# COMP6248-Reproducability-Challenge/selfsupervised-denoising

Hardware: AMD Instinct MI355X
Metric: training patches/sec (64x64 gauss25 SSDN) (higher is better)
Workload: dtype f16

## Files before the change

### selfsupervised-denoising_amd/csrc/conv_dma.hip

```cpp
#include "common.h"
#include <cstdlib>
#include <type_traits>
#include <utility>

#if defined(SSDN_CDMA_TUNING) || defined(SSDN_TUNING)
#define CD_ABL(xx, bit) (((xx).ablate & (bit)) != 0)
#define CD_TUNING 1
#else
#define CD_ABL(xx, bit) false
#define CD_TUNING 0
#endif

#ifndef CD_DEPHASE
#define CD_DEPHASE 0
#endif
#ifndef CD_MOVE_BARRIER
#define CD_MOVE_BARRIER 1
#endif
#ifndef CD_WARMUP
#define CD_WARMUP 1
#endif

namespace {

constexpr int CD_TBYTES = 31744;

struct CdAux {
    int m_base, m_cnt;
    int padT, padL, rev;
    int tiles_x, tiles_y;
    int segs, tps;
    int segs_sh;
    unsigned tx_magic;
    int nitems, xcd_map;
    int nfull, tail16;
    int ablate;
    int wrep;
    int dephase;
    unsigned long long* trace;
};

typedef __attribute__((address_space(3))) void* cd_lds_ptr;
__device__ __forceinline__ void dma16(unsigned lds_addr, int voff, __amdgpu_buffer_rsrc_t rs, int soff) {
    __builtin_amdgcn_raw_ptr_buffer_load_lds(rs, (cd_lds_ptr)(size_t)__builtin_amdgcn_readfirstlane(lds_addr), 16, voff, __builtin_amdgcn_readfirstlane(soff), 0, 0);
}

template <bool BF>
__device__ __forceinline__ void cd_mma(f32x16& c, half8 av, half8 bv) {
    if constexpr (BF) c = __builtin_amdgcn_mfma_f32_32x32x16_bf16(__builtin_bit_cast(bf16x8, av), __builtin_bit_cast(bf16x8, bv), c, 0, 0, 0);
    else c = __builtin_amdgcn_mfma_f32_32x32x16_f16(av, bv, c, 0, 0, 0);
}

template <int OFF>
__device__ __forceinline__ void lds_rd128(half8& dst, unsigned addr) {
    asm volatile("ds_read_b128 %0, %1 offset:%2" : "=v"(dst) : "v"(addr), "i"(OFF));
}
template <int MT>
__device__ __forceinline__ void lds_wait0(half8 (&aq)[MT], half8 (&bq)[2]) {
    if constexpr (MT == 3)
        asm volatile("s_waitcnt lgkmcnt(0)" : "+v"(aq[0]), "+v"(aq[1]), "+v"(aq[2]), "+v"(bq[0]), "+v"(bq[1]));
    else if constexpr (MT == 2)
        asm volatile("s_waitcnt lgkmcnt(0)" : "+v"(aq[0]), "+v"(aq[1]), "+v"(bq[0]), "+v"(bq[1]));
    else
        asm volatile("s_waitcnt lgkmcnt(0)" : "+v"(aq[0]), "+v"(bq[0]), "+v"(bq[1]));
}
template <int MT, int KS, int I, int J, int KS_>
__device__ __forceinline__ void cd_reads(half8 (&aq)[MT], half8 (&bq)[2], unsigned ap, unsigned bp) {
    constexpr int PSTR = KS * 32, PITCH = 18 * PSTR, BOFF = I * PITCH + J * PSTR;
    lds_rd128<BOFF + KS_ * 32>(bq[0], bp);
    lds_rd128<0 * 32 * PSTR + KS_ * 32>(aq[0], ap);
    lds_rd128<BOFF + 2 * PITCH + KS_ * 32>(bq[1], bp);
    if constexpr (MT > 1) lds_rd128<1 * 32 * PSTR + KS_ * 32>(aq[1], ap);
    if constexpr (MT > 2) lds_rd128<2 * 32 * PSTR + KS_ * 32>(aq[2], ap);
}
template <int MT, bool BF>
__device__ __forceinline__ void cd_mmas(f32x16 (&acc)[MT][2], const half8 (&aq)[MT], const half8 (&bq)[2]) {
#pragma unroll
    for (int mt = 0; mt < MT; ++mt) {
        cd_mma<BF>(acc[mt][0], aq[mt], bq[0]);
        cd_mma<BF>(acc[mt][1], aq[mt], bq[1]);
    }
}

struct CdTile { int n, y0, x0; };

template <int MT, bool FULL>
struct CdWSplit {
    static constexpr int nq = FULL ? MT * 3 : MT;
    static constexpr int NB = (nq + 1) / 2 > 4 ? 4 : (nq + 1) / 2;
    static constexpr bool extra = nq > 2 * NB;
    static constexpr int b1 = extra ? NB : nq - NB;
};
template <int N> using cd_ic = std::integral_constant<int, N>;
template <class F, int... Is>
__device__ __forceinline__ void cd_static_for_impl(F& f, std::integer_sequence<int, Is...>) { (f(cd_ic<Is>{}), ...); }
template <int N, class F>
__device__ __forceinline__ void cd_static_for(F&& f) { cd_static_for_impl(f, std::make_integer_sequence<int, N>{}); }
template <int IMM, int AUX = 0>
__device__ __forceinline__ void dma16i(unsigned lds_addr, int voff, __amdgpu_buffer_rsrc_t rs, int soff) {
    __builtin_amdgcn_raw_ptr_buffer_load_lds(rs, (cd_lds_ptr)(size_t)lds_addr, 16, voff, soff, IMM, AUX);
}

}

template <int MT, bool BF, int EPI, int KIND>
__global__ __launch_bounds__(256, 2) void k_cdma(ssdn_conv_args a, CdAux x) {
    constexpr bool AF = KIND == 1;
    extern __shared__ __attribute__((aligned(16))) char smem[];
    constexpr int WROWS = MT * 32;
    constexpr int WBYTES = WROWS * 96;
    constexpr int OSTR = MT * 64 + 16;
    constexpr int NEK = MT * 2;
    constexpr bool HAS_MASK = (EPI & 1) != 0, HAS_ADD = (EPI & 2) != 0, HAS_UPS = (EPI & 4) != 0, UROT = (EPI & 8) != 0;
    constexpr bool SOUT = (EPI & 16) != 0, SMASK = (EPI & 32) != 0;
    constexpr int NUK = (8 * MT * 4 + 63) / 64;
    constexpr int G = 2 * MT;
    constexpr bool MOVE = CD_MOVE_BARRIER != 0;
    const int tid = threadIdx.x, lane = tid & 63, l31 = lane & 31, kh = lane >> 5;
    const int w = __builtin_amdgcn_readfirstlane(tid >> 6);
    const bool wload = w < 2;
    const int lw = w & 1;
    const unsigned lds0 = (unsigned)(size_t)smem;
    char* const tbuf0 = smem;
    const unsigned tlds0 = lds0, wlds0 = lds0 + 2 * CD_TBYTES;

    const int G_ = gridDim.x;
    int it_first, it_stride, it_end;
    if (x.xcd_map) {
        const int i8 = x.nitems >> 3, xcd = blockIdx.x & 7;
        it_first = xcd * i8 + (blockIdx.x >> 3); it_stride = G_ >> 3; it_end = (xcd + 1) * i8;
    } else {
        it_first = blockIdx.x; it_stride = G_; it_end = x.nitems;
    }
    if (it_first >= it_end) return;
#if CD_WARMUP
    const int pf_line = (blockIdx.x >> 3) * 256 + tid;
    const unsigned pf = __builtin_amdgcn_raw_buffer_load_b32(
        __builtin_amdgcn_make_buffer_rsrc(const_cast<void*>(a.wc), 0, 9 * a.Mpad * a.Ktot * 2, SSDN_BUFFER_RSRC_FLAGS), pf_line << 7, 0, 0);
#endif

    const int bE48 = (4 * w + (l31 >> 4)) * 1728 + (l31 & 15) * 96 + ((kh ^ ((l31 >> 4) & 1)) << 4);
    const int aB48 = l31 * 96 + ((kh ^ ((l31 >> 3) & 1)) << 4);
    const int cpp = x.m_cnt >> 3;

    const __amdgpu_buffer_rsrc_t rs_wc = __builtin_amdgcn_make_buffer_rsrc(const_cast<void*>(a.wc), 0, (int)0x80000000, SSDN_BUFFER_RSRC_FLAGS);
    const int H0 = a.up0 ? (a.H >> 1) : a.H, W0 = a.up0 ? (a.W >> 1) : a.W;
    const int nch = x.nfull + x.tail16;

    int tr_i = 0;
    auto stamp = [&]() __attribute__((always_inline)) {
        if (CD_TUNING && x.trace && tid == 0 && tr_i < 32) x.trace[(size_t)blockIdx.x * 32 + tr_i++] = __builtin_amdgcn_s_memtime();
    };

    const int wtap = a.Mpad * a.Ktot * 2;
    const int wt0 = x.rev ? 8 * wtap : 0, wts = x.rev ? -wtap : wtap;
    const int wvoff = lane * 16;
    const bool lw0 = __builtin_amdgcn_readfirstlane(tid >> 6) == 0;
    auto wchunk = [&](int c) __attribute__((always_inline)) {
        return __builtin_amdgcn_readfirstlane((c * 48 * a.Mpad + x.m_base * ((AF || c < x.nfull) ? 48 : 16)) * 2 + wt0);
    };
    auto wpiece = [&](auto FULLc, auto Jc, unsigned d, int so) __attribute__((always_inline)) {
        using S = CdWSplit<MT, decltype(FULLc)::value != 0>;
        constexpr int j = decltype(Jc)::value;
        if (CD_ABL(x, 2)) return;
        if constexpr (j < S::NB) dma16i<j * 1024>(d, wvoff, rs_wc, so);
        else if constexpr (S::extra) { if (lw0) dma16i<0>(d + 2 * S::NB * 1024, wvoff, rs_wc, so + 2 * S::NB * 1024); }
    };
    auto wbase = [&](bool full) __attribute__((always_inline)) {
        return lw ? (full ? CdWSplit<MT, true>::b1 : CdWSplit<MT, false>::b1) * 1024 : 0;
    };
    auto wslice = [&](bool full, unsigned dbuf, int sl) __attribute__((always_inline)) {
        const int wb = wbase(full);
        if (AF || full) cd_static_for<CdWSplit<MT, true>::NB + 1>([&](auto jc) { wpiece(cd_ic<1>{}, jc, dbuf + wb, sl + wb); });
        else cd_static_for<CdWSplit<MT, false>::NB + 1>([&](auto jc) { wpiece(cd_ic<0>{}, jc, dbuf + wb, sl + wb); });
    };

    __amdgpu_buffer_rsrc_t rs_t = rs_wc;
    int t_so = 0, t_incA = 0, t_incB = 0, t_ybs = 0, rlE = 0, rlO = 0;
    unsigned t_tb = 0;
    auto tile_setup = [&](int tn, int ty0, int tx0, int c, int tbi, bool live) __attribute__((always_inline)) {
        const int k0 = c * 48;
        const bool from0 = k0 < a.c0;
        const bool up = from0 && a.up0;
        const int cs = from0 ? a.src0.cs : a.src1.cs;
        const int cbase = from0 ? a.src0.co + k0 : a.src1.co + k0 - a.c0;
        const int Hs = up ? H0 : a.H, Ws = up ? W0 : a.W;
        const bool full = AF || c < x.nfull;
        const int rstride = __builtin_amdgcn_readfirstlane(Ws * cs * 2);
        const int rbase = __builtin_amdgcn_readfirstlane(((CD_ABL(x, 128) ? 0 : tn) * Hs * Ws * cs + cbase) * 2);
        t_ybs = __builtin_amdgcn_readfirstlane(ty0 - x.padT);
        const int y_first = t_ybs + (full ? 0 : lw);
        t_so = rbase + (up ? y_first >> 1 : y_first) * rstride;
        t_incA = up ? ((y_first & 1) ? rstride : 0) : rstride;
        t_incB = up ? ((y_first & 1) ? 0 : rstride) : rstride;
        if (!full) { t_incA = up ? rstride : 2 * rstride; t_incB = t_incA; }
        t_tb = __builtin_amdgcn_readfirstlane(tlds0 + tbi * CD_TBYTES + (full ? lw * (44 * 16) : lw * 576));
        rs_t = __builtin_amdgcn_make_buffer_rsrc(from0 ? a.src0.p : (a.src1.p ? a.src1.p : a.src0.p), 0, live ? (int)0x80000000 : 0, SSDN_BUFFER_RSRC_FLAGS);
        const int rp = full ? lane + 44 * lw : lane;
        const int hp = rp / 6;
        const int hx = full ? hp : rp >> 1;
        const int cc = full ? rp - hp * 6 : rp & 1;
        const int xx = tx0 - x.padL + hx;
        const bool ok = (unsigned)xx < (unsigned)a.W;
        const int xs = up ? xx >> 1 : xx;
        rlE = ok ? (xs * cs + cc * 8) * 2 : (int)0x80000000;
        rlO = ok ? (xs * cs + (cc ^ 1) * 8) * 2 : (int)0x80000000;
    };
    auto trow = [&](auto FULLc, auto HYc) __attribute__((always_inline)) {
        constexpr bool full = decltype(FULLc)::value != 0;
        constexpr int hy = decltype(HYc)::value;
        if (CD_ABL(x, 4)) return;
        const int so = t_so;
        t_so += (hy & 1) ? t_incB : t_incA;
        if constexpr (full) {
            int voff = (hy & 1) ? rlO : rlE;
            if constexpr (hy < 2 || hy >= 16) voff = (unsigned)(t_ybs + hy) < (unsigned)a.H ? voff : (int)0x80000000;
            if (CD_ABL(x, 512)) dma16i<0, 2>(t_tb + hy * 1728, voff, rs_t, so);
            else dma16i<0>(t_tb + hy * 1728, voff, rs_t, so);
        } else {
            int voff = lw ? rlO : rlE;
            voff = (unsigned)(t_ybs + lw + 2 * hy) < (unsigned)a.H ? voff : (int)0x80000000;
            if (lane < 36) dma16i<0>(t_tb + hy * 1152, voff, rs_t, so);
        }
    };

    auto tile_of = [&](int item, int k) {
        const int strip = item >> x.segs_sh, seg = item & (x.segs - 1);
        CdTile t;
        t.n = x.tiles_x == 1 ? strip : (int)__umulhi((unsigned)strip, x.tx_magic);
        t.x0 = (strip - t.n * x.tiles_x) * 16;
        t.y0 = (seg * x.tps + k) * 16;
        return t;
    };
    int item = it_first, kt = 0;
    CdTile cur = tile_of(item, 0);
    int tpar = 0, wpar = 0;
    float* const bl = reinterpret_cast<float*>(smem + 18 * 18 * 96);
    if (tid < WROWS) bl[tid] = (a.bias && tid < x.m_cnt) ? a.bias[x.m_base + tid] : 0.f;
    constexpr int CD_LUT = 18 * 18 * 96 + 384;
    static_assert(CD_LUT + 256 <= CD_TBYTES && WROWS * 4 <= 384, "pad behind tile buffer 0");
    if constexpr (SMASK && HAS_MASK) {
        if (tid < 64) reinterpret_cast<float*>(smem + CD_LUT)[tid] = ((tid >> 2) >> (tid & 3)) & 1 ? 1.f : LRELU_SLOPE;
    }

    const __amdgpu_buffer_rsrc_t rs_dst = __builtin_amdgcn_make_buffer_rsrc(UROT ? a.urot.p : a.dst.p, 0, CD_ABL(x, 64) ? 0 : (int)0x80000000, SSDN_BUFFER_RSRC_FLAGS);
    const __amdgpu_buffer_rsrc_t rs_sgn = __builtin_amdgcn_make_buffer_rsrc(SOUT ? a.sign_out : a.urot_smask, 0, (!CD_ABL(x, 64) && (SOUT || (UROT && a.urot_smask))) ? (int)0x80000000 : 0, SSDN_BUFFER_RSRC_FLAGS);
    const __amdgpu_buffer_rsrc_t rs_ms = __builtin_amdgcn_make_buffer_rsrc(const_cast<void*>(HAS_UPS ? a.upsum_mask_sign : a.mask_sign), 0, SMASK ? (int)0x80000000 : 0, SSDN_BUFFER_RSRC_FLAGS);
    const float slope = a.act ? LRELU_SLOPE : 1.f;
    const __amdgpu_buffer_rsrc_t rs_mask = __builtin_amdgcn_make_buffer_rsrc(a.mask.p, 0, HAS_MASK ? (int)0x80000000 : 0, SSDN_BUFFER_RSRC_FLAGS);
    const __amdgpu_buffer_rsrc_t rs_add = __builtin_amdgcn_make_buffer_rsrc(a.add.p, 0, HAS_ADD ? (int)0x80000000 : 0, SSDN_BUFFER_RSRC_FLAGS);
    const __amdgpu_buffer_rsrc_t rs_up = __builtin_amdgcn_make_buffer_rsrc(a.upsum.p, 0, HAS_UPS ? (int)0x80000000 : 0, SSDN_BUFFER_RSRC_FLAGS);
    const __amdgpu_buffer_rsrc_t rs_um = __builtin_amdgcn_make_buffer_rsrc(a.upsum_mask.p, 0, HAS_UPS ? (int)0x80000000 : 0, SSDN_BUFFER_RSRC_FLAGS);
    int u_pc[NUK];
#pragma unroll
    for (int k = 0; k < NUK; ++k) {
        const int p = k * 64 + lane;
        const int j = p / cpp, c = p - j * cpp;
        u_pc[k] = p < 8 * cpp ? (j | (c << 8)) : -1;
    }

    auto run = [&](auto WLc) __attribute__((always_inline)) {
    constexpr bool WL = decltype(WLc)::value != 0;
    if constexpr (WL) {
        wslice(KIND != 0 || 0 < x.nfull, wlds0, wchunk(0));
        wslice(KIND != 0 || 0 < x.nfull, wlds0 + WBYTES, wchunk(0) + wts);
    } else {
        tile_setup(cur.n, cur.y0, cur.x0, 0, 0, true);
        if (KIND != 0 || 0 < x.nfull) cd_static_for<18>([&](auto hc) { trow(cd_ic<1>{}, hc); });
        else cd_static_for<9>([&](auto hc) { trow(cd_ic<0>{}, hc); });
    }
    asm volatile("s_waitcnt vmcnt(0)" ::: "memory");
    __builtin_amdgcn_s_barrier();
    if (CD_TUNING && x.trace && tid == 0) x.trace[(size_t)blockIdx.x * 32 + 31] = 0x100000000ull | (unsigned)__builtin_amdgcn_s_getreg((31 << 11) | 4);
    if (x.dephase > 0 && ((__builtin_amdgcn_s_getreg((31 << 11) | 4) >> 16) & 1))
        for (int d = 0; d < x.dephase; ++d) __builtin_amdgcn_s_sleep(16);
    stamp();
    for (;;) {
        int nitem = item, nkt = kt + 1;
        if (nkt >= x.tps) { nkt = 0; nitem = item + it_stride; }
        const bool has_next = nitem < it_end;
        const CdTile nxt = tile_of(has_next ? nitem : item, nkt);

        f32x16 acc[MT][2];
        int bo = kh * 16;
        asm volatile("" : "+v"(bo));
#pragma unroll
        for (int mt = 0; mt < MT; ++mt)
#pragma unroll
            for (int g = 0; g < 4; ++g) {
                const f32x4 bb = *reinterpret_cast<const f32x4*>(smem + 18 * 18 * 96 + (mt * 32 + g * 8) * 4 + bo);
#pragma unroll
                for (int j = 0; j < 4; ++j) { acc[mt][0][g * 4 + j] = bb[j]; acc[mt][1][g * 4 + j] = bb[j]; }
            }

        auto chunk = [&](int c, auto CFc, auto PFc) __attribute__((always_inline)) {
            constexpr int CF = decltype(CFc)::value, PFK = decltype(PFc)::value;
            const bool last_chunk = c + 1 == nch;
            const bool pf = !last_chunk || has_next;
            const int pc = last_chunk ? 0 : c + 1;
            const bool cfull = CF == 2 ? c < x.nfull : CF == 1, pf_full = PFK == 2 ? pc < x.nfull : PFK == 1;
            const unsigned tb = tlds0 + tpar * CD_TBYTES;
            int bE_ = bE48, aB_ = aB48;
            if (!cfull) {
                int lo = lane;
                asm volatile("" : "+v"(lo));
                const int l31o = lo & 31, kho = lo >> 5;
                bE_ = (4 * w + (l31o >> 4)) * 576 + (l31o & 15) * 32 + ((kho ^ ((l31o >> 4) & 1)) << 4);
                aB_ = l31o * 32 + ((kho ^ ((l31o >> 3) & 1)) << 4);
            }
            const unsigned bE = tb + bE_, bO = tb + (bE_ ^ 16);
            const unsigned apE = wlds0 + wpar * WBYTES + aB_, apO = wlds0 + (wpar ^ 1) * WBYTES + aB_;
            const bool wfirst = c == 0;
            int wso = 0;
            unsigned wdA = 0, wdB = 0;
            if constexpr (WL) {
                const int wb = wbase(cfull);
                wso = wchunk(c) + wb;
                wdA = __builtin_amdgcn_readfirstlane(wlds0 + wpar * WBYTES + wb);
                wdB = __builtin_amdgcn_readfirstlane(wlds0 + (wpar ^ 1) * WBYTES + wb);
            } else {
                tile_setup(last_chunk ? nxt.n : cur.n, last_chunk ? nxt.y0 : cur.y0, last_chunk ? nxt.x0 : cur.x0, pc, tpar ^ 1, pf);
            }
            auto body = [&](auto FULLc, auto PFULLc) __attribute__((always_inline)) {
                constexpr bool FULL = decltype(FULLc)::value != 0, PFULL = decltype(PFULLc)::value != 0;
                constexpr int KS = FULL ? 3 : 1;
                constexpr bool MV = MOVE && FULL && KIND != 0;
                half8 fa[2][MT], fb[2][2];
                auto gap = [&](auto Tc, auto Ic) __attribute__((always_inline)) {
                    constexpr int T = decltype(Tc)::value, i = decltype(Ic)::value;
                    if constexpr (WL) {
                        using S = CdWSplit<MT, FULL>;
                        constexpr int NP = S::NB + (S::extra ? 1 : 0);
                        if constexpr (T < 8) {
                            if constexpr (i == 0) wso += wts;
                            cd_static_for<NP>([&](auto jc) {
                                constexpr int j = decltype(jc)::value;
                                if constexpr ((j < G - 1 ? j : G - 1) == i) {
                                    if constexpr (T == 0) { if (!wfirst) wpiece(FULLc, jc, wdB, wso); }
                                    else wpiece(FULLc, jc, (T & 1) ? wdA : wdB, wso);
                                }
                            });
                        } else if constexpr (i == 0) {
                            if (pf) wslice(pf_full, wlds0 + (wpar ^ 1) * WBYTES, wchunk(pc));
                        }
                    } else {
                        constexpr int N = PFULL ? 18 : 9, NS = G >= 3 ? G : 3;
                        constexpr int k0 = T * NS, n = k0 >= N ? 0 : (N - k0 < NS ? N - k0 : NS);
                        cd_static_for<n>([&](auto kc) {
                            constexpr int k = decltype(kc)::value;
                            if constexpr ((k < G - 1 ? k : G - 1) == i) trow(PFULLc, cd_ic<k0 + k>{});
                        });
                    }
                };
// ... 4 lines not shown
                        if (wfirst && NEPI > 0 && cpp == 4 * MT && !CD_ABL(x, 8 | 1024)) asm volatile("s_waitcnt vmcnt(%0)" ::"n"(NEPI) : "memory");
                        else asm volatile("s_waitcnt vmcnt(0)" ::: "memory");
                    } else if (WL || T == 8) asm volatile("s_waitcnt vmcnt(0)" ::: "memory");
                    __builtin_amdgcn_s_barrier();
                };
                auto step = [&](auto Tc) __attribute__((always_inline)) {
                    constexpr int T = decltype(Tc)::value, I = T / 3, J = T % 3;
                    constexpr int P = MV ? (T & 1) : 0;
                    const unsigned ap = (T & 1) ? apO : apE, bp = (I & 1) ? bO : bE;
                    if constexpr (!MV || T == 0) cd_reads<MT, KS, I, J, 0>(fa[P], fb[P], ap, bp);
                    lds_wait0<MT>(fa[P], fb[P]);
                    if constexpr (KS > 1) cd_reads<MT, KS, I, J, 1>(fa[P ^ 1], fb[P ^ 1], ap, bp);
                    __builtin_amdgcn_sched_barrier(0);
                    cd_static_for<G>([&](auto ic) {
                        constexpr int i = decltype(ic)::value;
                        if (!CD_ABL(x, 1)) cd_mma<BF>(acc[i >> 1][i & 1], fa[P][i >> 1], fb[P][i & 1]);
                        __builtin_amdgcn_sched_barrier(0);
                        gap(Tc, ic);
                        __builtin_amdgcn_sched_barrier(0);
                    });
                    if constexpr (KS > 1) {
                        lds_wait0<MT>(fa[P ^ 1], fb[P ^ 1]);
                        cd_reads<MT, KS, I, J, 2>(fa[P], fb[P], ap, bp);
                        __builtin_amdgcn_sched_barrier(0);
                        if (!CD_ABL(x, 1)) cd_mmas<MT, BF>(acc, fa[P ^ 1], fb[P ^ 1]);
                        __builtin_amdgcn_sched_barrier(0);
                        lds_wait0<MT>(fa[P], fb[P]);
                        if constexpr (MV && T < 8) {
                            sync(Tc);
                            constexpr int T1 = T + 1, I1 = T1 / 3, J1 = T1 % 3;
                            cd_reads<MT, KS, I1, J1, 0>(fa[P ^ 1], fb[P ^ 1], (T1 & 1) ? apO : apE, (I1 & 1) ? bO : bE);
                            __builtin_amdgcn_sched_barrier(0);
                            if (!CD_ABL(x, 1)) cd_mmas<MT, BF>(acc, fa[P], fb[P]);
                            __builtin_amdgcn_sched_barrier(0);
                        } else {
                            if (!CD_ABL(x, 1)) cd_mmas<MT, BF>(acc, fa[P], fb[P]);
                            __builtin_amdgcn_sched_barrier(0);
                            sync(Tc);
                        }
                    } else sync(Tc);
                };
                step(cd_ic<0>{});
                stamp();
                cd_static_for<8>([&](auto tc) { step(cd_ic<decltype(tc)::value + 1>{}); });
            };
            if constexpr (CF != 2 && PFK != 2) body(cd_ic<CF>{}, cd_ic<PFK>{});
            else if constexpr (WL) {
                if (cfull) body(cd_ic<1>{}, cd_ic<1>{}); else body(cd_ic<0>{}, cd_ic<1>{});
            } else if (cfull) {
                if (pf_full) body(cd_ic<1>{}, cd_ic<1>{}); else body(cd_ic<1>{}, cd_ic<0>{});
            } else {
                if (pf_full) body(cd_ic<0>{}, cd_ic<1>{}); else body(cd_ic<0>{}, cd_ic<0>{});
            }
            tpar ^= 1; wpar ^= 1;
            stamp();
        };
        if constexpr (KIND == 1) {
            for (int c = 0; c < nch; ++c) chunk(c, cd_ic<1>{}, cd_ic<1>{});
        } else if constexpr (KIND == 2) {
            for (int c = 0; c + 1 < x.nfull; ++c) chunk(c, cd_ic<1>{}, cd_ic<1>{});
            chunk(x.nfull - 1, cd_ic<1>{}, cd_ic<0>{});
            chunk(x.nfull, cd_ic<0>{}, cd_ic<1>{});
        } else {
            for (int c = 0; c < nch; ++c) chunk(c, cd_ic<2>{}, cd_ic<2>{});
        }
        if constexpr (WL) {
            if (has_next) wslice(KIND != 0 || 0 < x.nfull, wlds0 + (wpar ^ 1) * WBYTES, wchunk(0) + wts);
        }
        if (!CD_ABL(x, 8) && !HAS_UPS && (cpp & 1) == 0 && !CD_ABL(x, 1024)) {
            const int pix_t = (cur.n * a.H + cur.y0 + 4 * w) * a.W + cur.x0;
            const int npair = __builtin_amdgcn_readfirstlane(cpp >> 1);
            int lane_o = lane;
            asm volatile("" : "+v"(lane_o));
            const int l31 = lane_o & 31, kh = lane_o >> 5;
            const int lrow = l31 >> 4, lcol = l31 & 15;
            const int lpix = lrow * a.W + lcol;
            int ur_base = 0, ur_iu = 0, ur_iv = 0, ur_ju = 0, ur_jv = 0;
            if constexpr (UROT) {
                const int Bq = a.N >> 2, P1 = a.H - 1;
                const int r = (cur.n >= Bq ? 1 : 0) + (cur.n >= 2 * Bq ? 1 : 0) + (cur.n >= 3 * Bq ? 1 : 0);
                ur_iu = r == 0 ? 1 : (r == 2 ? -1 : 0); ur_iv = r == 1 ? 1 : (r == 3 ? -1 : 0);
                ur_ju = r == 3 ? 1 : (r == 1 ? -1 : 0); ur_jv = r == 0 ? 1 : (r == 2 ? -1 : 0);
                const int i0 = r >= 2 ? P1 : 0, j0 = (r == 1 || r == 2) ? P1 : 0;
                ur_base = (((cur.n - r * Bq) * a.H + i0) * a.W + j0) * a.urot.cs + a.urot.co + r * a.M;
            }
            constexpr bool HOIST = HAS_MASK && SMASK && !HAS_ADD && !UROT;
            unsigned mbh[2][MT * 2];
            if constexpr (HOIST) {
#pragma unroll
                for (int nt = 0; nt < 2; ++nt) {
                    const int pix_p = pix_t + 2 * nt * a.W;
                    const int s_so = __builtin_amdgcn_readfirstlane(pix_p * (a.M >> 3) + (x.m_base >> 3));
#pragma unroll
                    for (int i = 0; i < MT * 2; ++i) {
                        if (i >= npair) break;
                        mbh[nt][i] = __builtin_amdgcn_raw_buffer_load_b8(rs_ms, lpix * (a.M >> 3) + kh + i * 2, s_so, 0);
                    }
                }
            }
            auto pass = [&](auto NtC, auto ActC) __attribute__((always_inline)) {
                constexpr int nt = decltype(NtC)::value;
                constexpr bool ACTC = decltype(ActC)::value != 0;
                const int pix_p = pix_t + 2 * nt * a.W;
                int d_lane, d_so = 0;
                bool live = true;
                if constexpr (UROT) {
                    const int u = cur.y0 + 4 * w + 2 * nt + lrow + 1, v = cur.x0 + lcol;
                    live = u < a.H;
                    const int dpx = (ur_iu * u + ur_iv * v) * a.W + ur_ju * u + ur_jv * v;
                    d_lane = live ? (ur_base + dpx * a.urot.cs + x.m_base) * 2 + kh * 16 : (int)0x80000000;
                } else {
                    d_lane = lpix * a.dst.cs * 2 + kh * 16;
                    d_so = __builtin_amdgcn_readfirstlane((pix_p * a.dst.cs + a.dst.co + x.m_base) * 2);
                }
                const int s_lane = live ? lpix * (a.M >> 3) + kh : (int)0x80000000;
                const int s_so = __builtin_amdgcn_readfirstlane(pix_p * (a.M >> 3) + (x.m_base >> 3));
                u32x4_t ab[MT * 2], mb[MT * 2];
#pragma unroll
                for (int i = 0; i < MT * 2; ++i) {
                    if (i >= npair) break;
                    if constexpr (HAS_ADD)
                        ab[i] = __builtin_amdgcn_raw_buffer_load_b128(rs_add, lpix * a.add.cs * 2 + kh * 16 + i * 32,
                                                                      __builtin_amdgcn_readfirstlane((pix_p * a.add.cs + a.add.co + x.m_base) * 2), 0);
                    if constexpr (HOIST)
                        mb[i][0] = mbh[nt][i];
                    else if constexpr (HAS_MASK && SMASK)
                        mb[i][0] = __builtin_amdgcn_raw_buffer_load_b8(rs_ms, s_lane + i * 2, s_so, 0);
                    else if constexpr (HAS_MASK)
                        mb[i] = __builtin_amdgcn_raw_buffer_load_b128(rs_mask, lpix * a.mask.cs * 2 + kh * 16 + i * 32,
                                                                      __builtin_amdgcn_readfirstlane((pix_p * a.mask.cs + a.mask.co + x.m_base) * 2), 0);
                }
#pragma unroll
                for (int mt = 0; mt < MT; ++mt)
#pragma unroll
                    for (int gp = 0; gp < 2; ++gp) {
                        constexpr int DUMMY = 0; (void)DUMMY;
                        const int i = mt * 2 + gp;
                        if (i >= npair) break;
                        unsigned pk[2][2];
#pragma unroll
                        for (int h = 0; h < 2; ++h) {
                            float v[4];
#pragma unroll
                            for (int j = 0; j < 4; ++j) v[j] = acc[mt][nt][(2 * gp + h) * 4 + j];
                            if constexpr (ACTC) {
#pragma unroll
                                for (int j = 0; j < 4; j += 2) {
                                    const f32x2_t t = f32x2_t{v[j], v[j + 1]} * LRELU_SLOPE;
                                    asm("v_max_f32 %0, %1, %2" : "=v"(v[j]) : "v"(v[j]), "v"(t[0]));
                                    asm("v_max_f32 %0, %1, %2" : "=v"(v[j + 1]) : "v"(v[j + 1]), "v"(t[1]));
                                }
                            }
                            pk[h][0] = BF ? pack_bf16x2(v[0], v[1]) : pack_f16x2(v[0], v[1]);
                            pk[h][1] = BF ? pack_bf16x2(v[2], v[3]) : pack_f16x2(v[2], v[3]);
                        }
                        u32x4_t o;
#pragma unroll
                        for (int d = 0; d < 2; ++d) {
                            auto r = __builtin_amdgcn_permlane32_swap(pk[0][d], pk[1][d], false, false);
                            o[d] = r[0]; o[2 + d] = r[1];
                        }
                        if constexpr (HAS_MASK && SMASK && BF) {
                            const unsigned sb = mb[i][0];
                            const f32x4 m0 = *reinterpret_cast<const f32x4*>(smem + CD_LUT + ((sb & 15u) << 4));
                            const f32x4 m1 = *reinterpret_cast<const f32x4*>(smem + CD_LUT + ((sb >> 4) << 4));
#pragma unroll
                            for (int q = 0; q < 4; ++q) {
                                f32x2_t v = f32x2_t{bf_lo(o[q]), bf_hi(o[q])};
                                if constexpr (HAS_ADD) v = v + f32x2_t{bf_lo(ab[i][q]), bf_hi(ab[i][q])};
                                v = v * (q < 2 ? f32x2_t{m0[2 * q], m0[2 * q + 1]} : f32x2_t{m1[2 * q - 4], m1[2 * q - 3]});
                                o[q] = pack_bf16x2(v[0], v[1]);
                            }
                        } else if constexpr (HAS_MASK || HAS_ADD) {
#pragma unroll
                            for (int q = 0; q < 4; ++q) {
                                float v0, v1;
                                if constexpr (BF) {
                                    v0 = bf_lo(o[q]); v1 = bf_hi(o[q]);
                                    if constexpr (HAS_ADD) { v0 += bf_lo(ab[i][q]); v1 += bf_hi(ab[i][q]); }
                                } else {
                                    v0 = f16_lo(o[q]); v1 = f16_hi(o[q]);
                                    if constexpr (HAS_ADD) { v0 += f16_lo(ab[i][q]); v1 += f16_hi(ab[i][q]); }
                                }
                                if constexpr (HAS_MASK) {
                                    int mlo, mhi;
                                    if constexpr (SMASK) { mlo = (mb[i][0] >> (2 * q)) & 1u; mhi = (mb[i][0] >> (2 * q + 1)) & 1u; }
                                    else { mlo = (int)(short)(mb[i][q] & 0xffffu); mhi = (int)mb[i][q] >> 16; }
                                    v0 *= mlo > 0 ? 1.f : LRELU_SLOPE;
                                    v1 *= mhi > 0 ? 1.f : LRELU_SLOPE;
                                }
                                o[q] = BF ? pack_bf16x2(v0, v1) : pack_f16x2(v0, v1);
                            }
                        }
                        if (CD_ABL(x, 256)) __builtin_amdgcn_raw_buffer_store_b128(o, rs_dst, d_lane + i * 32, d_so, 2);
                        else __builtin_amdgcn_raw_buffer_store_b128(o, rs_dst, d_lane + i * 32, d_so, 0);
                        asm volatile("s_nop 7" ::: "memory");
                        if constexpr (UROT || SOUT) {
                            if (SOUT || a.urot_smask) {
                                unsigned rq[4];
#pragma unroll
                                for (int q = 0; q < 4; ++q) {
                                    unsigned t0;
                                    asm("v_pk_max_i16 %0, %1, 0" : "=v"(t0) : "v"(o[q]));
                                    asm("v_pk_min_i16 %0, %1, %2" : "=v"(rq[q]) : "v"(t0), "s"(0x00010001u));
                                }
                                const unsigned t01 = (rq[1] << 2) | rq[0], t23 = (rq[3] << 2) | rq[2];
                                const unsigned t = (t23 << 4) | t01;
                                const unsigned sb = t | (t >> 15);
                                __builtin_amdgcn_raw_buffer_store_b8((unsigned char)sb, rs_sgn, s_lane + i * 2, s_so, 0);
                            }
                        }
                    }
            };
            if (a.act) { pass(std::integral_constant<int, 0>{}, std::integral_constant<int, 1>{}); pass(std::integral_constant<int, 1>{}, std::integral_constant<int, 1>{}); }
            else { pass(std::integral_constant<int, 0>{}, std::integral_constant<int, 0>{}); pass(std::integral_constant<int, 1>{}, std::integral_constant<int, 0>{}); }
        } else
        if (!CD_ABL(x, 8)) {
            char* reg = tbuf0 + (tpar ^ 1) * CD_TBYTES + w * (32 * OSTR);
            const int pix_t = (cur.n * a.H + cur.y0 + 4 * w) * a.W + cur.x0;
            int lane_o = lane;
            asm volatile("" : "+v"(lane_o));
            const int l31 = lane_o & 31, kh = lane_o >> 5;
            int e_pc[NEK];
            if constexpr (!HAS_UPS) {
#pragma unroll
                for (int k = 0; k < NEK; ++k) {
                    const int p = k * 64 + lane_o;
                    const int px = p / cpp, c = p - px * cpp;
                    e_pc[k] = p < 32 * cpp ? (px | (c << 8)) : -1;
                }
            } else {
#pragma unroll
                for (int k = 0; k < NEK; ++k) e_pc[k] = -1;
            }
            int ur_base = 0, ur_iu = 0, ur_iv = 0, ur_ju = 0, ur_jv = 0;
            if constexpr (UROT) {
                const int Bq = a.N >> 2, P1 = a.H - 1;
                const int r = (cur.n >= Bq ? 1 : 0) + (cur.n >= 2 * Bq ? 1 : 0) + (cur.n >= 3 * Bq ? 1 : 0);
                ur_iu = r == 0 ? 1 : (r == 2 ? -1 : 0); ur_iv = r == 1 ? 1 : (r == 3 ? -1 : 0);
                ur_ju = r == 3 ? 1 : (r == 1 ? -1 : 0); ur_jv = r == 0 ? 1 : (r == 2 ? -1 : 0);
                const int i0 = r >= 2 ? P1 : 0, j0 = (r == 1 || r == 2) ? P1 : 0;
                ur_base = (((cur.n - r * Bq) * a.H + i0) * a.W + j0) * a.urot.cs + a.urot.co + r * a.M;
            }
#pragma unroll
            for (int nt = 0; nt < 2; ++nt) {
                const int pix_p = pix_t + 2 * nt * a.W;
                u32x4_t ab[NEK], mb[NEK];
                int goff[NEK], soff[NEK];
#pragma unroll
                for (int k = 0; k < NEK; ++k) {
                    int epc = e_pc[k];
                    asm volatile("" : "+v"(epc));
                    const bool on = epc >= 0;
                    const int px = epc & 255, c16 = (epc >> 8) << 4;
                    const int pix = pix_p + (px >> 4) * a.W + (px & 15);
                    if constexpr (UROT) {
                        const int u = cur.y0 + 4 * w + 2 * nt + (px >> 4) + 1, v = cur.x0 + (px & 15);
                        const bool live = on && u < a.H;
                        const int dpx = (ur_iu * u + ur_iv * v) * a.W + ur_ju * u + ur_jv * v;
                        goff[k] = live ? (ur_base + dpx * a.urot.cs + x.m_base) * 2 + c16 : (int)0x80000000;
                        soff[k] = live ? pix * (a.M >> 3) + (x.m_base >> 3) + (c16 >> 4) : (int)0x80000000;
                    } else
                    goff[k] = on ? (pix * a.dst.cs + a.dst.co + x.m_base) * 2 + c16 : (int)0x80000000;
                    if constexpr (HAS_ADD)
                        ab[k] = __builtin_amdgcn_raw_buffer_load_b128(rs_add, on ? (pix * a.add.cs + a.add.co + x.m_base) * 2 + c16 : (int)0x80000000, 0, 0);
                    if constexpr (HAS_MASK && SMASK)
                        mb[k][0] = __builtin_amdgcn_raw_buffer_load_b8(rs_ms, on ? pix * (a.M >> 3) + (x.m_base >> 3) + (c16 >> 4) : (int)0x80000000, 0, 0);
                    else if constexpr (HAS_MASK)
                        mb[k] = __builtin_amdgcn_raw_buffer_load_b128(rs_mask, on ? (pix * a.mask.cs + a.mask.co + x.m_base) * 2 + c16 : (int)0x80000000, 0, 0);
                    if constexpr (SOUT) soff[k] = on ? pix * (a.M >> 3) + (x.m_base >> 3) + (c16 >> 4) : (int)0x80000000;
// ... 57 lines not shown
                        }
                        u32x4_t r;
#pragma unroll
                        for (int q = 0; q < 4; ++q) {
                            int mlo, mhi;
                            if constexpr (SMASK) { mlo = (um[k][0] >> (2 * q)) & 1u; mhi = (um[k][0] >> (2 * q + 1)) & 1u; }
                            else { mlo = (int)(short)(um[k][q] & 0xffffu); mhi = (int)um[k][q] >> 16; }
                            r[q] = pack_bf16x2(sum[2 * q] * (mlo > 0 ? 1.f : LRELU_SLOPE), sum[2 * q + 1] * (mhi > 0 ? 1.f : LRELU_SLOPE));
                        }
                        __builtin_amdgcn_raw_buffer_store_b128(r, rs_up, on ? ((pixl + j) * a.upsum.cs + a.upsum.co + x.m_base) * 2 + c16 : (int)0x80000000, 0, 0);
                    }
                } else {
#pragma unroll
                for (int k = 0; k < NEK; ++k) {
                    int epc = e_pc[k];
                    asm volatile("" : "+v"(epc));
                    const bool on = epc >= 0;
                    const int px = epc & 255, c16 = (epc >> 8) << 4;
                    u32x4_t o = *reinterpret_cast<const u32x4_t*>(reg + (on ? px * OSTR + c16 : 0));
                    if constexpr (HAS_MASK || HAS_ADD) {
#pragma unroll
                        for (int q = 0; q < 4; ++q) {
                            float v0, v1;
                            if constexpr (BF) {
                                v0 = bf_lo(o[q]); v1 = bf_hi(o[q]);
                                if constexpr (HAS_ADD) { v0 += bf_lo(ab[k][q]); v1 += bf_hi(ab[k][q]); }
                            } else {
                                v0 = f16_lo(o[q]); v1 = f16_hi(o[q]);
                                if constexpr (HAS_ADD) { v0 += f16_lo(ab[k][q]); v1 += f16_hi(ab[k][q]); }
                            }
                            if constexpr (HAS_MASK) {
                                int mlo, mhi;
                                if constexpr (SMASK) { mlo = (mb[k][0] >> (2 * q)) & 1u; mhi = (mb[k][0] >> (2 * q + 1)) & 1u; }
                                else { mlo = (int)(short)(mb[k][q] & 0xffffu); mhi = (int)mb[k][q] >> 16; }
                                v0 *= mlo > 0 ? 1.f : LRELU_SLOPE;
                                v1 *= mhi > 0 ? 1.f : LRELU_SLOPE;
                            }
                            o[q] = BF ? pack_bf16x2(v0, v1) : pack_f16x2(v0, v1);
                        }
                    }
                    __builtin_amdgcn_raw_buffer_store_b128(o, rs_dst, goff[k], 0, 0);
                    if constexpr (UROT || SOUT) {
                        if (SOUT || a.urot_smask) {
                            unsigned sb = 0;
#pragma unroll
                            for (int q = 0; q < 4; ++q)
                                sb |= ((int)(short)(o[q] & 0xffffu) > 0 ? 1u : 0u) << (2 * q) | (((int)o[q] >> 16) > 0 ? 1u : 0u) << (2 * q + 1);
                            __builtin_amdgcn_raw_buffer_store_b8((unsigned char)sb, rs_sgn, soff[k], 0, 0);
                        }
                    }
                }
                }
            }
        }
        stamp();
        if (!has_next) break;
        if (CD_ABL(x, 1024) || HAS_UPS || (cpp & 1)) __builtin_amdgcn_s_barrier();
        item = nitem; kt = nkt; cur = nxt;
    }
    };
    if (wload) run(cd_ic<1>{}); else run(cd_ic<0>{});
#if CD_WARMUP
    asm volatile("" :: "v"(pf));
#endif
}

#ifndef CD_KERNEL_ONLY
static bool cd_window(const ssdn_conv_args* a, int* padT, int* padL, int* rev) {
    if (a->ntaps != 9) return false;
    int mny = 0, mnx = 0;
    for (int t = 0; t < 9; ++t) { mny = a->dy[t] < mny ? a->dy[t] : mny; mnx = a->dx[t] < mnx ? a->dx[t] : mnx; }
    bool fwd = true, mir = true;
    for (int t = 0; t < 9; ++t) {
        const int i = a->dy[t] - mny, j = a->dx[t] - mnx;
        if (i != t / 3 || j != t % 3) fwd = false;
        if (i != 2 - t / 3 || j != 2 - t % 3) mir = false;
    }
    if (!fwd && !mir) return false;
    *padT = -mny; *padL = -mnx; *rev = fwd ? 0 : 1;
    return true;
}

bool conv_dma_eligible(const ssdn_conv_args* a, bool any_size) {
    int pt, pl, rv;
    if (!cd_window(a, &pt, &pl, &rv)) return false;
    if (a->dst32 || (a->H & 15) || (a->W & 15) || !a->wc) return false;
    const int tail = a->Ktot % 48;
    if (tail != 0 && tail != 16) return false;
    if (a->c0 % 48 && a->c0 != a->Ktot) return false;
    if ((a->M & 7) || (a->Mpad & 31)) return false;
    if (!a->bf16 && (a->mask.p || a->add.p)) return false;
    if (a->bf16 && a->act) return false;
    if (a->urot.p && (a->bf16 || a->M != 96 || a->Mpad != 96 || a->H != a->W || (a->N & 3) || a->mask.p || a->add.p || a->upsum.p || a->pool.p ||
                      (a->urot.co & 7) || (a->urot.cs & 7) || (long long)(a->N / 4) * a->H * a->W * a->urot.cs * 2 >= (1ll << 31))) return false;
    if (a->upsum.p && (!a->bf16 || a->mask.p || a->add.p || a->upsum_c % 96 || a->upsum_c > a->M)) return false;
    int cus = ssdn_device_cus();
    if (cus <= 0) cus = 256;
    const long long tiles = (long long)a->N * (a->H >> 4) * (a->W >> 4);
    if (!(tiles >= cus || (2 * tiles >= cus && a->H * a->W > 256)) && !any_size) return false;
    if ((long long)a->N * (a->W >> 4) >= 65536) return false;
    int csmax = a->dst.cs > a->src1.cs ? a->dst.cs : a->src1.cs;
    csmax = csmax > a->src0.cs ? csmax : a->src0.cs;
    csmax = csmax > a->mask.cs ? csmax : a->mask.cs;
    csmax = csmax > a->add.cs ? csmax : a->add.cs;
    if ((long long)a->N * a->H * a->W * csmax * 2 >= (1ll << 31)) return false;
    if (9ll * a->Mpad * a->Ktot * 2 >= (1ll << 31)) return false;
    return true;
}

bool conv_dma_signs(const ssdn_conv_args* a) {
    if (!conv_dma_eligible(a, false)) return false;
    if (a->sign_out && (a->bf16 || !a->dst.p || a->urot.p || a->M != 96 || a->Mpad != 96)) return false;
    if (a->mask_sign && (!a->bf16 || !a->mask.p || a->add.p || a->upsum.p || a->mask.cs != a->M || a->mask.co != 0 || (a->Mpad != 96 && a->Mpad != 64))) return false;
    if (a->upsum_mask_sign && (!a->bf16 || !a->upsum.p || a->upsum_mask.cs != a->upsum_c || a->upsum_mask.co != 0)) return false;
    return true;
}

int conv_dma_lds_bytes(int mt) { return 2 * CD_TBYTES + 2 * mt * 32 * 96; }

template <int MT, bool BF, int EPI, int KIND>
static int cd_launch_kind(const ssdn_conv_args* a, CdAux x, hipStream_t s) {
    static bool attr_set_dev[SSDN_MAX_DEVICES_ATTR] = {};
    bool& attr_set = attr_set_dev[ssdn_current_device_slot()];
    if (!attr_set) {
        SSDN_CHECK_HIP(hipFuncSetAttribute((const void*)k_cdma<MT, BF, EPI, KIND>, hipFuncAttributeMaxDynamicSharedMemorySize, 160 * 1024));
        attr_set = true;
    }
    int cus = ssdn_device_cus();
    if (cus <= 0) return -1;
    const int nstrips = a->N * x.tiles_x;
    x.segs = 1;
    while (nstrips * x.segs < 2 * cus && x.segs < x.tiles_y && x.tiles_y % (x.segs * 2) == 0) x.segs *= 2;
    x.tps = x.tiles_y / x.segs;
    x.segs_sh = 0;
    while ((1 << x.segs_sh) < x.segs) ++x.segs_sh;
    x.tx_magic = x.tiles_x > 1 ? (unsigned)((0x100000000ull + x.tiles_x - 1) / x.tiles_x) : 0u;
    x.nitems = nstrips * x.segs;
    const int grid = x.nitems < 2 * cus ? x.nitems : 2 * cus;
    x.xcd_map = (x.nitems % 8 == 0 && grid % 8 == 0) ? 1 : 0;
    const double px = (double)a->N * a->H * a->W;
    const int kreal = a->kreal > 0 ? a->kreal : a->Ktot;
    const double flops = 2.0 * px * x.m_cnt * kreal * 9;
    const double bytes = px * (a->c0 * 2.0 / (a->up0 ? 4.0 : 1.0) + a->c1 * 2.0) + px * x.m_cnt * 2.0;
    prof_begin(MT == 3 ? SSDN_PROF_CDMA_MT3 : SSDN_PROF_CDMA_MT21, s);
    SSDN_LAUNCH((k_cdma<MT, BF, EPI, KIND>), dim3(grid), dim3(256), conv_dma_lds_bytes(MT), s, *a, x);
    prof_end(MT == 3 ? SSDN_PROF_CDMA_MT3 : SSDN_PROF_CDMA_MT21, s, flops, bytes);
    return 0;
}
template <int MT, bool BF, int EPI>
static int cd_launch(const ssdn_conv_args* a, const CdAux& x, hipStream_t s) {
    if (x.tail16 == 0 && x.nfull > 0) return cd_launch_kind<MT, BF, EPI, 1>(a, x, s);
    if constexpr (!BF) {
        if (x.tail16 == 1 && x.nfull > 0) return cd_launch_kind<MT, BF, EPI, 2>(a, x, s);
    }
    return cd_launch_kind<MT, BF, EPI, 0>(a, x, s);
}

template <int MT>
static int cd_launch_role(const ssdn_conv_args* a, const CdAux& x, hipStream_t s) {
    if (a->urot.p) {
        if constexpr (MT == 3) return cd_launch<3, false, 8>(a, x, s);
        return ssdn_set_error("conv_dma: fused UNROT_FWD needs M = 96");
    }
    if (!a->bf16) {
        if (a->sign_out) {
            if constexpr (MT == 3) return cd_launch<3, false, 16>(a, x, s);
            return ssdn_set_error("conv_dma: sign_out needs M = 96");
        }
        return cd_launch<MT, false, 0>(a, x, s);
    }
    if (a->upsum.p && x.m_base < a->upsum_c) {
        if constexpr (MT == 3) {
            if (x.m_base + 96 <= a->upsum_c && x.m_cnt == 96 && !a->mask.p && !a->add.p)
                return a->upsum_mask_sign ? cd_launch<3, true, 4 | 32>(a, x, s) : cd_launch<3, true, 4>(a, x, s);
        }
        return ssdn_set_error("conv_dma: fused upsum needs whole 96-channel blocks without mask / add");
    }
    const int epi = (a->mask.p ? 1 : 0) | (a->add.p ? 2 : 0);
    if (a->mask_sign) {
        if constexpr (MT >= 2) { if (epi == 1) return cd_launch<MT, true, 1 | 32>(a, x, s); }
        return ssdn_set_error("conv_dma: mask_sign needs a mask, no skip gradient, Mpad = 96 or 64");
    }
    switch (epi) {
        case 0: return cd_launch<MT, true, 0>(a, x, s);
        case 1: return cd_launch<MT, true, 1>(a, x, s);
        case 2: return cd_launch<MT, true, 2>(a, x, s);
        default: return cd_launch<MT, true, 3>(a, x, s);
    }
}

int launch_conv_dma(const ssdn_conv_args* a, hipStream_t s) {
    CdAux x;
    if (!cd_window(a, &x.padT, &x.padL, &x.rev)) return ssdn_set_error("conv_dma: not a 3x3 window");
    x.tiles_x = a->W >> 4; x.tiles_y = a->H >> 4;
    x.segs = 1; x.tps = x.tiles_y; x.nitems = 0; x.xcd_map = 0; x.segs_sh = 0; x.tx_magic = 0;
    x.nfull = a->Ktot / 48; x.tail16 = (a->Ktot % 48) ? 1 : 0;
    static const int env_ablate = [] { const char* e = ssdn_tuning_env("SSDN_CDMA_ABLATE"); return e ? atoi(e) : 0; }();
    x.ablate = env_ablate;
    static const int env_wrep = [] { const char* e = ssdn_tuning_env("SSDN_CDMA_WREP"); return e ? atoi(e) : 0; }();
    x.wrep = env_wrep;
    static const int env_dephase = [] { const char* e = ssdn_tuning_env("SSDN_CDMA_DEPHASE"); return e ? atoi(e) : CD_DEPHASE; }();
    x.dephase = env_dephase;
    x.trace = (unsigned long long*)ssdn_debug_get_trace();
// ... 19 lines not shown
```

Measured before the change: 20600.

## Add 48-channel conv kernel variant using 16x16x32 MFMA tiles

Adds a KIND 3 path of the DMA conv kernel for 48-output-channel layers. It uses 16x16x32 MFMA instructions instead of padding to 64 rows with 32x32 tiles. The path has its own weight LDS layout, tap schedule, and read/prefetch interleaving, plus a direct epilogue using permlane16 swaps. The goal is to remove wasted MFMA work and weight traffic from padding 48 channels to 64. The cost is more code paths and a different LDS footprint for MT=2 launches.

```diff
diff --git a/selfsupervised-denoising_amd/csrc/conv_dma.hip b/selfsupervised-denoising_amd/csrc/conv_dma.hip
--- a/selfsupervised-denoising_amd/csrc/conv_dma.hip
+++ b/selfsupervised-denoising_amd/csrc/conv_dma.hip
@@ -50,6 +50,16 @@
     if constexpr (BF) c = __builtin_amdgcn_mfma_f32_32x32x16_bf16(__builtin_bit_cast(bf16x8, av), __builtin_bit_cast(bf16x8, bv), c, 0, 0, 0);
     else c = __builtin_amdgcn_mfma_f32_32x32x16_f16(av, bv, c, 0, 0, 0);
 }
+template <bool BF>
+__device__ __forceinline__ void cd_mma16(f32x4& c, half8 av, half8 bv) {
+    if constexpr (BF) c = __builtin_amdgcn_mfma_f32_16x16x32_bf16(__builtin_bit_cast(bf16x8, av), __builtin_bit_cast(bf16x8, bv), c, 0, 0, 0);
+    else c = __builtin_amdgcn_mfma_f32_16x16x32_f16(av, bv, c, 0, 0, 0);
+}
+
+constexpr int CD48_W = 48 * 96;
+constexpr int CD48_LDS = 2 * CD_TBYTES + 4 * CD48_W;
+__host__ __device__ constexpr int cd48_ta(int s) { return s == 0 ? 0 : s == 1 ? 3 : s == 2 ? 6 : s == 3 ? 2 : 8; }
+__host__ __device__ constexpr int cd48_tb(int s) { return s == 0 ? 1 : s == 1 ? 4 : s == 2 ? 7 : s == 3 ? 5 : -1; }
 
 template <int OFF>
 __device__ __forceinline__ void lds_rd128(half8& dst, unsigned addr) {
@@ -72,6 +82,9 @@
     lds_rd128<BOFF + 2 * PITCH + KS_ * 32>(bq[1], bp);
     if constexpr (MT > 1) lds_rd128<1 * 32 * PSTR + KS_ * 32>(aq[1], ap);
     if constexpr (MT > 2) lds_rd128<2 * 32 * PSTR + KS_ * 32>(aq[2], ap);
+}
+__device__ __forceinline__ void lds_wait48(half8 (&aq)[3], half8 (&bq)[4]) {
+    asm volatile("s_waitcnt lgkmcnt(0)" : "+v"(aq[0]), "+v"(aq[1]), "+v"(aq[2]), "+v"(bq[0]), "+v"(bq[1]), "+v"(bq[2]), "+v"(bq[3]));
 }
 template <int MT, bool BF>
 __device__ __forceinline__ void cd_mmas(f32x16 (&acc)[MT][2], const half8 (&aq)[MT], const half8 (&bq)[2]) {
@@ -105,7 +118,9 @@
 
 template <int MT, bool BF, int EPI, int KIND>
 __global__ __launch_bounds__(256, 2) void k_cdma(ssdn_conv_args a, CdAux x) {
-    constexpr bool AF = KIND == 1;
+    constexpr bool U48 = KIND == 3;
+    static_assert(!U48 || (MT == 2 && (EPI & (4 | 8 | 16)) == 0), "KIND 3: 48 rows, direct epilogue");
+    constexpr bool AF = KIND == 1 || U48;
     extern __shared__ __attribute__((aligned(16))) char smem[];
     constexpr int WROWS = MT * 32;
     constexpr int WBYTES = WROWS * 96;
@@ -173,6 +188,22 @@
         const int wb = wbase(full);
         if (AF || full) cd_static_for<CdWSplit<MT, true>::NB + 1>([&](auto jc) { wpiece(cd_ic<1>{}, jc, dbuf + wb, sl + wb); });
         else cd_static_for<CdWSplit<MT, false>::NB + 1>([&](auto jc) { wpiece(cd_ic<0>{}, jc, dbuf + wb, sl + wb); });
+    };
+    auto w48piece = [&](auto Jc, unsigned d, int so) __attribute__((always_inline)) {
+        constexpr int j = decltype(Jc)::value;
+        if (CD_ABL(x, 2)) return;
+        if constexpr (j < 4) dma16i<j * 1024>(d, wvoff, rs_wc, so);
+        else if (lane < 32) dma16i<0>(d + 4096, wvoff, rs_wc, so + 4096);
+    };
+    auto w48dst = [&](auto Sc, int wc, unsigned pd, unsigned& d, int& so) __attribute__((always_inline)) {
+        constexpr int S = decltype(Sc)::value;
+        d = __builtin_amdgcn_readfirstlane(pd + lw * CD48_W);
+        so = __builtin_amdgcn_readfirstlane(wc + (lw ? cd48_tb(S) : cd48_ta(S)) * wts);
+        return S < 4 || lw == 0;
+    };
+    auto w48slice = [&](auto Sc, int wc, unsigned pd) __attribute__((always_inline)) {
+        unsigned d; int so;
+        if (w48dst(Sc, wc, pd, d, so)) cd_static_for<5>([&](auto jc) { w48piece(jc, d, so); });
     };
 
     __amdgpu_buffer_rsrc_t rs_t = rs_wc;
@@ -261,7 +292,10 @@
 
     auto run = [&](auto WLc) __attribute__((always_inline)) {
     constexpr bool WL = decltype(WLc)::value != 0;
-    if constexpr (WL) {
+    if constexpr (WL && U48) {
+        w48slice(cd_ic<0>{}, wchunk(0), wlds0);
+        w48slice(cd_ic<1>{}, wchunk(0), wlds0 + 2 * CD48_W);
+    } else if constexpr (WL) {
         wslice(KIND != 0 || 0 < x.nfull, wlds0, wchunk(0));
         wslice(KIND != 0 || 0 < x.nfull, wlds0 + WBYTES, wchunk(0) + wts);
     } else {
@@ -281,7 +315,17 @@
         const bool has_next = nitem < it_end;
         const CdTile nxt = tile_of(has_next ? nitem : item, nkt);
 
-        f32x16 acc[MT][2];
+        std::conditional_t<U48, f32x4[3][4], f32x16[MT][2]> acc;
+        if constexpr (U48) {
+            int bo = (lane >> 4) * 16;
+            asm volatile("" : "+v"(bo));
+#pragma unroll
+            for (int mt = 0; mt < 3; ++mt) {
+                const f32x4 bb = *reinterpret_cast<const f32x4*>(smem + 18 * 18 * 96 + mt * 64 + bo);
+#pragma unroll
+                for (int r = 0; r < 4; ++r) acc[mt][r] = bb;
+            }
+        } else {
         int bo = kh * 16;
         asm volatile("" : "+v"(bo));
 #pragma unroll
@@ -292,13 +336,103 @@
 #pragma unroll
                 for (int j = 0; j < 4; ++j) { acc[mt][0][g * 4 + j] = bb[j]; acc[mt][1][g * 4 + j] = bb[j]; }
             }
+        }
+
+        auto chunk48 = [&](auto , int c, bool pf, int pc) __attribute__((always_inline)) {
+            const bool wfirst = c == 0;
+            int lo = lane;
+            asm volatile("" : "+v"(lo));
+            const int qo = lo >> 4, no = lo & 15, mp = (lo >> 3) & 1;
+            const unsigned bb = tlds0 + tpar * CD_TBYTES + 4 * w * 1728 + no * 96;
+            unsigned b0[2], b1h[2], b1v[2], b2[2];
+#pragma unroll
+            for (int p = 0; p < 2; ++p) {
+                b0[p] = bb + ((qo ^ p) << 4);
+                b1h[p] = bb + (qo < 2 ? ((4 + qo) ^ p) << 4 : 96 + (((qo - 2) ^ p) << 4));
+                b1v[p] = bb + (qo < 2 ? ((4 + qo) ^ p) << 4 : 1728 + (((qo - 2) ^ p ^ 1) << 4));
+                b2[p] = bb + (((2 + qo) ^ p) << 4);
+            }
+            const unsigned fa0 = no * 96 + ((qo ^ mp) << 4);
+            const unsigned fa1 = no * 96 + (qo < 2 ? ((4 + qo) ^ mp) << 4 : CD48_W + (((qo - 2) ^ mp) << 4));
+            const unsigned fa2 = no * 96 + CD48_W + (((2 + qo) ^ mp) << 4);
+            const unsigned pE = wlds0 + wpar * 2 * CD48_W, pO = wlds0 + (wpar ^ 1) * 2 * CD48_W;
+            const unsigned aE[3] = {pE + fa0, pE + fa1, pE + fa2}, aO[3] = {pO + fa0, pO + fa1, pO + fa2};
+            half8 fa[2][3], fb[2][4];
+            auto reads = [&](auto Sc, auto Uc, auto Fc) __attribute__((always_inline)) {
+                constexpr int S = decltype(Sc)::value, U = decltype(Uc)::value, F = decltype(Fc)::value;
+                constexpr int t = U == 2 ? cd48_tb(S) : cd48_ta(S), I = t / 3, J = t % 3;
+                cd_static_for<4>([&](auto rc) {
+                    constexpr int r = decltype(rc)::value, p = (r + I) & 1;
+                    const unsigned bp = U == 0 ? b0[p] : U == 2 ? b2[p] : S == 3 ? b1v[p] : b1h[p];
+                    lds_rd128<(r + I) * 1728 + J * 96>(fb[F][r], bp);
+                    if constexpr (r < 3) lds_rd128<r * 1536>(fa[F][r], (S & 1) ? aO[U] : aE[U]);
+                });
+            };
+            auto sync = [&](auto Tc) __attribute__((always_inline)) {
+                constexpr int T = decltype(Tc)::value;
+                if constexpr (WL && T == 0) {
+                    constexpr int NEPI = 6 * (1 + (HAS_ADD ? 1 : 0) + (HAS_MASK ? 1 : 0));
+                    if (wfirst && !CD_ABL(x, 8 | 1024)) asm volatile("s_waitcnt vmcnt(%0)" ::"n"(NEPI) : "memory");
+                    else asm volatile("s_waitcnt vmcnt(0)" ::: "memory");
+                } else if (WL || T == 4) asm volatile("s_waitcnt vmcnt(0)" ::: "memory");
+                __builtin_amdgcn_s_barrier();
+            };
+            auto step = [&](auto Tc) __attribute__((always_inline)) {
+                constexpr int T = decltype(Tc)::value, NK = T < 4 ? 3 : 2, K0 = 3 * T;
+                unsigned wd = 0;
+                int wso = 0;
+                bool wlive = false;
+                if constexpr (WL) {
+                    if constexpr (T < 4) wlive = !(T == 0 && wfirst) && w48dst(cd_ic<T + 1>{}, wchunk(c), wlds0 + (wpar ^ ((T + 1) & 1)) * 2 * CD48_W, wd, wso);
+                    else wlive = pf && w48dst(cd_ic<0>{}, wchunk(pc), wlds0 + (wpar ^ 1) * 2 * CD48_W, wd, wso);
+                }
+                if constexpr (T == 0) reads(cd_ic<0>{}, cd_ic<0>{}, cd_ic<0>{});
+                cd_static_for<NK>([&](auto uc) {
+                    constexpr int u = decltype(uc)::value, F = (K0 + u) & 1;
+                    lds_wait48(fa[F], fb[F]);
+                    if constexpr (T == 4 && u == 1) {
+                        if (lo >= 32) {
+#pragma unroll
+                            for (int k = 0; k < 3; ++k) fa[F][k] = half8{};
+#pragma unroll
+                            for (int k = 0; k < 4; ++k) fb[F][k] = half8{};
+                        }
+                    }
+                    if constexpr (u + 1 < NK) reads(cd_ic<T>{}, cd_ic<u + 1>{}, cd_ic<F ^ 1>{});
+                    else if constexpr (T < 4) {
+                        sync(Tc);
+                        reads(cd_ic<T + 1>{}, cd_ic<0>{}, cd_ic<F ^ 1>{});
+                    }
+                    __builtin_amdgcn_sched_barrier(0);
+                    cd_static_for<12>([&](auto ic) {
+                        constexpr int i = decltype(ic)::value;
+                        if constexpr (U48) { if (!CD_ABL(x, 1)) cd_mma16<BF>(acc[i >> 2][i & 3], fa[F][i >> 2], fb[F][i & 3]); }
+                        __builtin_amdgcn_sched_barrier(0);
+                        if constexpr (u == 0) {
+                            if constexpr (WL) {
+                                if constexpr (i < 5) { if (wlive) w48piece(ic, wd, wso); }
+                            } else if constexpr (T < 3 && i < 6) trow(cd_ic<1>{}, cd_ic<T * 6 + i>{});
+                            __builtin_amdgcn_sched_barrier(0);
+                        }
+                    });
+                });
+                if constexpr (T == 4) sync(Tc);
+            };
+            step(cd_ic<0>{});
+            stamp();
+            cd_static_for<4>([&](auto tc) { step(cd_ic<decltype(tc)::value + 1>{}); });
+        };
 
         auto chunk = [&](int c, auto CFc, auto PFc) __attribute__((always_inline)) {
             constexpr int CF = decltype(CFc)::value, PFK = decltype(PFc)::value;
             const bool last_chunk = c + 1 == nch;
             const bool pf = !last_chunk || has_next;
             const int pc = last_chunk ? 0 : c + 1;
-            const bool cfull = CF == 2 ? c < x.nfull : CF == 1, pf_full = PFK == 2 ? pc < x.nfull : PFK == 1;
+            if constexpr (U48) {
+                if constexpr (!WL) tile_setup(last_chunk ? nxt.n : cur.n, last_chunk ? nxt.y0 : cur.y0, last_chunk ? nxt.x0 : cur.x0, pc, tpar ^ 1, pf);
+                chunk48(cd_ic<3>{}, c, pf, pc);
+            } else {
+            const bool cfull =CF == 2 ? c < x.nfull : CF == 1, pf_full = PFK == 2 ? pc < x.nfull : PFK == 1;
             const unsigned tb = tlds0 + tpar * CD_TBYTES;
             int bE_ = bE48, aB_ = aB48;
             if (!cfull) {
@@ -409,10 +543,11 @@
             } else {
                 if (pf_full) body(cd_ic<0>{}, cd_ic<1>{}); else body(cd_ic<0>{}, cd_ic<0>{});
             }
+            }
             tpar ^= 1; wpar ^= 1;
             stamp();
         };
-        if constexpr (KIND == 1) {
+        if constexpr (KIND == 1 || U48) {
             for (int c = 0; c < nch; ++c) chunk(c, cd_ic<1>{}, cd_ic<1>{});
         } else if constexpr (KIND == 2) {
             for (int c = 0; c + 1 < x.nfull; ++c) chunk(c, cd_ic<1>{}, cd_ic<1>{});
@@ -421,7 +556,9 @@
         } else {
             for (int c = 0; c < nch; ++c) chunk(c, cd_ic<2>{}, cd_ic<2>{});
         }
-        if constexpr (WL) {
+        if constexpr (WL && U48) {
+            if (has_next) w48slice(cd_ic<1>{}, wchunk(0), wlds0 + (wpar ^ 1) * 2 * CD48_W);
+        } else if constexpr (WL) {
             if (has_next) wslice(KIND != 0 || 0 < x.nfull, wlds0 + (wpar ^ 1) * WBYTES, wchunk(0) + wts);
         }
         if (!CD_ABL(x, 8) && !HAS_UPS && (cpp & 1) == 0 && !CD_ABL(x, 1024)) {
@@ -488,18 +625,18 @@
                                                                       __builtin_amdgcn_readfirstlane((pix_p * a.mask.cs + a.mask.co + x.m_base) * 2), 0);
                 }
 #pragma unroll
-                for (int mt = 0; mt < MT; ++mt)
-#pragma unroll
-                    for (int gp = 0; gp < 2; ++gp) {
-                        constexpr int DUMMY = 0; (void)DUMMY;
-                        const int i = mt * 2 + gp;
+                for (int i = 0; i < (U48 ? 3 : MT * 2); ++i) {
                         if (i >= npair) break;
+                        const int mt = U48 ? i : i >> 1, gp = i & 1;
                         unsigned pk[2][2];
 #pragma unroll
                         for (int h = 0; h < 2; ++h) {
                             float v[4];
 #pragma unroll
-                            for (int j = 0; j < 4; ++j) v[j] = acc[mt][nt][(2 * gp + h) * 4 + j];
+                            for (int j = 0; j < 4; ++j) {
+                                if constexpr (U48) v[j] = acc[mt][2 * nt + h][j];
+                                else v[j] = acc[mt][nt][(2 * gp + h) * 4 + j];
+                            }
                             if constexpr (ACTC) {
 #pragma unroll
                                 for (int j = 0; j < 4; j += 2) {
@@ -514,8 +651,13 @@
                         u32x4_t o;
 #pragma unroll
                         for (int d = 0; d < 2; ++d) {
-                            auto r = __builtin_amdgcn_permlane32_swap(pk[0][d], pk[1][d], false, false);
-                            o[d] = r[0]; o[2 + d] = r[1];
+                            if constexpr (U48) {
+                                auto r = __builtin_amdgcn_permlane16_swap(pk[0][d], pk[1][d], false, false);
+                                o[d] = r[0]; o[2 + d] = r[1];
+                            } else {
+                                auto r = __builtin_amdgcn_permlane32_swap(pk[0][d], pk[1][d], false, false);
+                                o[d] = r[0]; o[2 + d] = r[1];
+                            }
                         }
                         if constexpr (HAS_MASK && SMASK && BF) {
                             const unsigned sb = mb[i][0];
@@ -572,7 +714,8 @@
             if (a.act) { pass(std::integral_constant<int, 0>{}, std::integral_constant<int, 1>{}); pass(std::integral_constant<int, 1>{}, std::integral_constant<int, 1>{}); }
             else { pass(std::integral_constant<int, 0>{}, std::integral_constant<int, 0>{}); pass(std::integral_constant<int, 1>{}, std::integral_constant<int, 0>{}); }
         } else
-        if (!CD_ABL(x, 8)) {
+        if (!U48 && !CD_ABL(x, 8)) {
+          if constexpr (!U48) {
             char* reg = tbuf0 + (tpar ^ 1) * CD_TBYTES + w * (32 * OSTR);
             const int pix_t = (cur.n * a.H + cur.y0 + 4 * w) * a.W + cur.x0;
             int lane_o = lane;
@@ -736,6 +879,7 @@
                 }
                 }
             }
+          }
         }
         stamp();
         if (!has_next) break;
@@ -800,7 +944,7 @@
     return true;
 }
 
-int conv_dma_lds_bytes(int mt) { return 2 * CD_TBYTES + 2 * mt * 32 * 96; }
+int conv_dma_lds_bytes(int mt) { return mt == 2 ? CD48_LDS : 2 * CD_TBYTES + 2 * mt * 32 * 96; }
 
 template <int MT, bool BF, int EPI, int KIND>
 static int cd_launch_kind(const ssdn_conv_args* a, CdAux x, hipStream_t s) {
@@ -827,12 +971,15 @@
     const double flops = 2.0 * px * x.m_cnt * kreal * 9;
     const double bytes = px * (a->c0 * 2.0 / (a->up0 ? 4.0 : 1.0) + a->c1 * 2.0) + px * x.m_cnt * 2.0;
     prof_begin(MT == 3 ? SSDN_PROF_CDMA_MT3 : SSDN_PROF_CDMA_MT21, s);
-    SSDN_LAUNCH((k_cdma<MT, BF, EPI, KIND>), dim3(grid), dim3(256), conv_dma_lds_bytes(MT), s, *a, x);
+    SSDN_LAUNCH((k_cdma<MT, BF, EPI, KIND>), dim3(grid), dim3(256), KIND == 3 ? CD48_LDS : 2 * CD_TBYTES + 2 * MT * 32 * 96, s, *a, x);
     prof_end(MT == 3 ? SSDN_PROF_CDMA_MT3 : SSDN_PROF_CDMA_MT21, s, flops, bytes);
     return 0;
 }
 template <int MT, bool BF, int EPI>
 static int cd_launch(const ssdn_conv_args* a, const CdAux& x, hipStream_t s) {
+    if constexpr (MT == 2 && (EPI & (4 | 8 | 16)) == 0) {
+        if (x.tail16 == 0 && x.nfull > 0 && x.m_cnt == 48) return cd_launch_kind<2, BF, EPI, 3>(a, x, s);
+    }
     if (x.tail16 == 0 && x.nfull > 0) return cd_launch_kind<MT, BF, EPI, 1>(a, x, s);
     if constexpr (!BF) {
         if (x.tail16 == 1 && x.nfull > 0) return cd_launch_kind<MT, BF, EPI, 2>(a, x, s);
```

After: 20740, median of 6. No clear change (+0.7%).
